# xymeng16/dcf

Hardware: AMD Instinct MI355X
Metric: DCF evals/sec (node) at 128-bit input, λ=16B; AES blocks/s vs INT roofline (higher is better)
Workload: dtype u8

## Files before the change

### dcf_amd/csrc/aes_lds.h

```cpp
#pragma once

namespace {

uint8_t g_sbox[256];
uint32_t g_tab[4 * 256];
std::once_flag g_aes_once;

uint8_t gmul(uint8_t a, uint8_t b) {
  uint8_t r = 0;
  for (; b; b >>= 1) {
    if (b & 1) r ^= a;
    a = (uint8_t)((a << 1) ^ ((a & 0x80) ? 0x1b : 0));
  }
  return r;
}

void aes_init_tables() {
  uint8_t exp_t[256], log_t[256] = {0};
  uint8_t x = 1;
  for (int i = 0; i < 255; i++) {
    exp_t[i] = x;
    log_t[x] = (uint8_t)i;
    x = gmul(x, 3);
  }
  for (int v = 0; v < 256; v++) {
    uint8_t inv = v ? exp_t[(255 - log_t[v]) % 255] : 0;
    uint8_t s = inv;
    for (int k = 1; k <= 4; k++) s ^= (uint8_t)((inv << k) | (inv >> (8 - k)));
    g_sbox[v] = (uint8_t)(s ^ 0x63);
  }
  for (int v = 0; v < 256; v++) {
    uint32_t s = g_sbox[v], s2 = gmul((uint8_t)s, 2), s3 = gmul((uint8_t)s, 3);
    uint32_t t0 = s2 | (s << 8) | (s << 16) | (s3 << 24);
    for (int t = 0; t < 4; t++) g_tab[t * 256 + v] = t ? ((t0 << (8 * t)) | (t0 >> (32 - 8 * t))) : t0;
  }
}

struct RoundKeys {
  uint32_t w[60];
};

void aes256_expand_words(const uint8_t key[32], RoundKeys* rk) {
  uint8_t b[240];
  memcpy(b, key, 32);
  uint8_t rcon = 1;
  for (int i = 8; i < 60; i++) {
    uint8_t t[4] = {b[4 * i - 4], b[4 * i - 3], b[4 * i - 2], b[4 * i - 1]};
    if (i % 8 == 0) {
      uint8_t t0 = t[0];
      t[0] = (uint8_t)(g_sbox[t[1]] ^ rcon);
      t[1] = g_sbox[t[2]];
      t[2] = g_sbox[t[3]];
      t[3] = g_sbox[t0];
      rcon = gmul(rcon, 2);
    } else if (i % 8 == 4) {
      for (auto& c : t) c = g_sbox[c];
    }
    for (int k = 0; k < 4; k++) b[4 * i + k] = (uint8_t)(b[4 * (i - 8) + k] ^ t[k]);
  }
  for (int i = 0; i < 60; i++)
    rk->w[i] = (uint32_t)b[4 * i] | ((uint32_t)b[4 * i + 1] << 8) | ((uint32_t)b[4 * i + 2] << 16) |
               ((uint32_t)b[4 * i + 3] << 24);
}

void aes128_expand_words(const uint8_t key[16], uint32_t w[44]) {
  uint8_t b[176];
  memcpy(b, key, 16);
  uint8_t rcon = 1;
  for (int i = 4; i < 44; i++) {
    uint8_t t[4] = {b[4 * i - 4], b[4 * i - 3], b[4 * i - 2], b[4 * i - 1]};
    if (i % 4 == 0) {
      const uint8_t t0 = t[0];
      t[0] = (uint8_t)(g_sbox[t[1]] ^ rcon);
      t[1] = g_sbox[t[2]];
      t[2] = g_sbox[t[3]];
      t[3] = g_sbox[t0];
      rcon = gmul(rcon, 2);
    }
    for (int k = 0; k < 4; k++) b[4 * i + k] = (uint8_t)(b[4 * (i - 4) + k] ^ t[k]);
  }
  for (int i = 0; i < 44; i++)
    w[i] = (uint32_t)b[4 * i] | ((uint32_t)b[4 * i + 1] << 8) | ((uint32_t)b[4 * i + 2] << 16) |
           ((uint32_t)b[4 * i + 3] << 24);
}

constexpr int kLdsWords = 32768;
constexpr int kBlock = 1024;
constexpr uint32_t kMaskLast = 0xFEFFFFFFu;

__device__ __forceinline__ void lds_fill_tables(uint32_t* lds, const uint32_t* __restrict__ tab) {
  for (int idx = threadIdx.x; idx < kLdsWords; idx += blockDim.x) {
    const int half = idx >> 14, rem = idx & 16383;
    const int b = rem >> 6, slot = rem & 63;
    lds[idx] = tab[(2 * half + (slot >> 5)) * 256 + b];
  }
  __syncthreads();
}

__device__ __forceinline__ uint32_t lane_const() {
  const uint32_t l = (threadIdx.x & 31u) * 4u;
  return l | ((128u + l) << 8) | (1u << 16);
}

template <int T, int K>
struct Sel {
  static constexpr uint32_t v =
      ((T & 1) ? 1u : 0u) | ((4u + K) << 8) | (((T >> 1) ? 2u : 0x0cu) << 16) | (0x0cu << 24);
};

#ifndef DCF_T1_BITOP3
#define DCF_T1_BITOP3 1
#endif
template <int T, int K, bool B1 = true>
__device__ __forceinline__ uint32_t lk(const uint32_t* lds, uint32_t w, uint32_t lc) {
  uint32_t addr;
  if (DCF_T1_BITOP3 && B1 && T == 1 && K == 1) {
    addr = __builtin_amdgcn_bitop3_b32(w, 0xFF00u, (lc >> 8) & 0xFFu, 0xEA);
  } else {
    addr = __builtin_amdgcn_perm(w, lc, Sel<T, K>::v);
  }
  return *reinterpret_cast<const uint32_t*>(reinterpret_cast<const char*>(lds) + addr);
}

constexpr int kQpRot1 = 1 | (2 << 2) | (3 << 4) | (0 << 6);
constexpr int kQpRot2 = 2 | (3 << 2) | (0 << 4) | (1 << 6);
constexpr int kQpRot3 = 3 | (0 << 2) | (1 << 4) | (2 << 6);
constexpr int kQpBcast0 = 0;

__device__ __forceinline__ uint32_t xor3(uint32_t a, uint32_t b, uint32_t c) {
  return __builtin_amdgcn_bitop3_b32(a, b, c, 0x96);
}

template <int NB>
__device__ __forceinline__ void aes256_tt(uint32_t (&st)[NB][4], const RoundKeys& rk, const uint32_t* lds,
                                          uint32_t lc) {
#pragma unroll
  for (int b = 0; b < NB; ++b)
#pragma unroll
    for (int j = 0; j < 4; ++j) st[b][j] ^= rk.w[j];
#pragma unroll
  for (int r = 1; r < 14; ++r) {
    uint32_t o[NB][4];
#pragma unroll
    for (int b = 0; b < NB; ++b)
#pragma unroll
      for (int j = 0; j < 4; ++j) {
        const uint32_t a = lk<0, 0>(lds, st[b][j], lc);
        const uint32_t c = lk<1, 1>(lds, st[b][(j + 1) & 3], lc);
        const uint32_t d = lk<2, 2>(lds, st[b][(j + 2) & 3], lc);
        const uint32_t e = lk<3, 3>(lds, st[b][(j + 3) & 3], lc);
        o[b][j] = xor3(xor3(a, c, d), e, rk.w[4 * r + j]);
      }
#pragma unroll
    for (int b = 0; b < NB; ++b)
#pragma unroll
      for (int j = 0; j < 4; ++j) st[b][j] = o[b][j];
  }
  uint32_t o[NB][4];
#pragma unroll
  for (int b = 0; b < NB; ++b)
#pragma unroll
    for (int j = 0; j < 4; ++j) {
      const uint32_t a = lk<2, 0>(lds, st[b][j], lc);
      const uint32_t c = lk<3, 1>(lds, st[b][(j + 1) & 3], lc);
      const uint32_t d = lk<0, 2>(lds, st[b][(j + 2) & 3], lc);
      const uint32_t e = lk<1, 3>(lds, st[b][(j + 3) & 3], lc);
      const uint32_t lo = __builtin_amdgcn_perm(c, a, 0x0c0c0500u);
      const uint32_t hi = __builtin_amdgcn_perm(e, d, 0x07020c0cu);
      o[b][j] = xor3(lo, hi, rk.w[56 + j]);
    }
#pragma unroll
  for (int b = 0; b < NB; ++b)
#pragma unroll
    for (int j = 0; j < 4; ++j) st[b][j] = o[b][j];
}

typedef unsigned int u32x4_t __attribute__((ext_vector_type(4)));
__device__ __forceinline__ uint4 lds_load16(uint32_t a) {
  const u32x4_t v = *(__attribute__((address_space(3))) const u32x4_t*)(size_t)a;
  return make_uint4(v.x, v.y, v.z, v.w);
}

template <int NR, int NB, bool PRE, int KR = 0>
__device__ __forceinline__ void aes_tt_lka(uint32_t (&st)[NB][4], const uint32_t (&ka)[NB], const uint32_t* lds,
                                           uint32_t lc, const uint32_t (*rkr)[2][4] = nullptr,
                                           const uint32_t* hm = nullptr) {
  if (!PRE) {
#pragma unroll
    for (int b = 0; b < NB; ++b) {
      const uint4 k = lds_load16(ka[b]);
      st[b][0] ^= k.x; st[b][1] ^= k.y; st[b][2] ^= k.z; st[b][3] ^= k.w;
    }
  }
#pragma unroll
  for (int r = 1; r <= NR; ++r) {
    uint32_t o[NB][4];
#pragma unroll
    for (int b = 0; b < NB; ++b) {
      uint32_t kw[4];
      if (r < KR) {
#pragma unroll
        for (int j = 0; j < 4; ++j) kw[j] = __builtin_amdgcn_bitop3_b32(hm[b], rkr[r][1][j], rkr[r][0][j], 0xCA);
      } else {
        const uint4 k = lds_load16(ka[b] + 16u * r);
        kw[0] = k.x; kw[1] = k.y; kw[2] = k.z; kw[3] = k.w;
      }
#pragma unroll
      for (int j = 0; j < 4; ++j) {
        if (r < NR) {
          const uint32_t a = lk<0, 0, false>(lds, st[b][j], lc);
          const uint32_t c = lk<1, 1, false>(lds, st[b][(j + 1) & 3], lc);
          const uint32_t d = lk<2, 2, false>(lds, st[b][(j + 2) & 3], lc);
          const uint32_t e = lk<3, 3, false>(lds, st[b][(j + 3) & 3], lc);
          o[b][j] = xor3(xor3(a, c, d), e, kw[j]);
        } else {
          const uint32_t a = lk<2, 0>(lds, st[b][j], lc);
          const uint32_t c = lk<3, 1>(lds, st[b][(j + 1) & 3], lc);
          const uint32_t d = lk<0, 2>(lds, st[b][(j + 2) & 3], lc);
          const uint32_t e = lk<1, 3>(lds, st[b][(j + 3) & 3], lc);
          o[b][j] = xor3(__builtin_amdgcn_perm(c, a, 0x0c0c0500u), __builtin_amdgcn_perm(e, d, 0x07020c0cu), kw[j]);
        }
      }
    }
#pragma unroll
    for (int b = 0; b < NB; ++b)
#pragma unroll
      for (int j = 0; j < 4; ++j) st[b][j] = o[b][j];
  }
}

template <int NR, int NB, bool LATE_KEYS = false>
__device__ __forceinline__ void aes_tt_lk(uint32_t (&st)[NB][4], const uint4* const (&rk)[NB], const uint32_t* lds,
                                          uint32_t lc) {
#pragma unroll
  for (int b = 0; b < NB; ++b) {
    const uint4 k = rk[b][0];
    st[b][0] ^= k.x; st[b][1] ^= k.y; st[b][2] ^= k.z; st[b][3] ^= k.w;
  }
#pragma unroll
  for (int r = 1; r < NR; ++r) {
    uint32_t o[NB][4];
#pragma unroll
    for (int b = 0; b < NB; ++b) {
      uint32_t z = 0u;
      if (LATE_KEYS) asm volatile("" : "+v"(z) : "v"(st[b][0]));
      const uint4 k = rk[b][r + z];
      const uint32_t kw[4] = {k.x, k.y, k.z, k.w};
#pragma unroll
      for (int j = 0; j < 4; ++j) {
        const uint32_t a = lk<0, 0>(lds, st[b][j], lc);
        const uint32_t c = lk<1, 1>(lds, st[b][(j + 1) & 3], lc);
        const uint32_t d = lk<2, 2>(lds, st[b][(j + 2) & 3], lc);
        const uint32_t e = lk<3, 3>(lds, st[b][(j + 3) & 3], lc);
        o[b][j] = xor3(xor3(a, c, d), e, kw[j]);
      }
    }
#pragma unroll
    for (int b = 0; b < NB; ++b)
#pragma unroll
      for (int j = 0; j < 4; ++j) st[b][j] = o[b][j];
  }
  uint32_t o[NB][4];
#pragma unroll
  for (int b = 0; b < NB; ++b) {
    const uint4 k = rk[b][NR];
    const uint32_t kw[4] = {k.x, k.y, k.z, k.w};
#pragma unroll
    for (int j = 0; j < 4; ++j) {
      const uint32_t a = lk<2, 0>(lds, st[b][j], lc);
      const uint32_t c = lk<3, 1>(lds, st[b][(j + 1) & 3], lc);
      const uint32_t d = lk<0, 2>(lds, st[b][(j + 2) & 3], lc);
      const uint32_t e = lk<1, 3>(lds, st[b][(j + 3) & 3], lc);
      const uint32_t lo = __builtin_amdgcn_perm(c, a, 0x0c0c0500u);
      const uint32_t hi = __builtin_amdgcn_perm(e, d, 0x07020c0cu);
      o[b][j] = xor3(lo, hi, kw[j]);
    }
  }
#pragma unroll
  for (int b = 0; b < NB; ++b)
#pragma unroll
    for (int j = 0; j < 4; ++j) st[b][j] = o[b][j];
}

template <int NB, bool PRE = false>
__device__ __forceinline__ void aes256_tt_gk(uint32_t (&st)[NB][4], const uint4* __restrict__ rkg,
                                             const uint32_t* lds, uint32_t lc) {
  const char* base = reinterpret_cast<const char*>(rkg);
  uint32_t zb = 0u;
  if (!PRE) {
    const uint4 k = *reinterpret_cast<const uint4*>(base);
#pragma unroll
    for (int b = 0; b < NB; ++b) {
      st[b][0] ^= k.x; st[b][1] ^= k.y; st[b][2] ^= k.z; st[b][3] ^= k.w;
    }
  }
  constexpr int AH = 3;
  uint4 kq[AH];
#pragma unroll
  for (int q = 0; q < AH - 1; ++q) kq[q] = *reinterpret_cast<const uint4*>(base + 16 * (q + 1));
#pragma unroll
  for (int r = 1; r < 15; ++r) {
    asm volatile("" : "+v"(zb) : "v"(st[0][0]), "v"(st[NB - 1][0]));
    const int rn = r + AH - 1;
    if (rn < 15) kq[(rn - 1) % AH] = *reinterpret_cast<const uint4*>(base + zb + 16 * rn);
    const uint4 k = kq[(r - 1) % AH];
    const uint32_t kw[4] = {k.x, k.y, k.z, k.w};
    uint32_t o[NB][4];
    if (r < 14) {
#pragma unroll
      for (int b = 0; b < NB; ++b)
#pragma unroll
        for (int j = 0; j < 4; ++j) {
          const uint32_t a = lk<0, 0>(lds, st[b][j], lc);
          const uint32_t c = lk<1, 1>(lds, st[b][(j + 1) & 3], lc);
          const uint32_t d = lk<2, 2>(lds, st[b][(j + 2) & 3], lc);
          const uint32_t e = lk<3, 3>(lds, st[b][(j + 3) & 3], lc);
          o[b][j] = xor3(xor3(a, c, d), e, kw[j]);
        }
    } else {
#pragma unroll
      for (int b = 0; b < NB; ++b)
#pragma unroll
        for (int j = 0; j < 4; ++j) {
          const uint32_t a = lk<2, 0>(lds, st[b][j], lc);
          const uint32_t c = lk<3, 1>(lds, st[b][(j + 1) & 3], lc);
          const uint32_t d = lk<0, 2>(lds, st[b][(j + 2) & 3], lc);
          const uint32_t e = lk<1, 3>(lds, st[b][(j + 3) & 3], lc);
          const uint32_t lo = __builtin_amdgcn_perm(c, a, 0x0c0c0500u);
          const uint32_t hi = __builtin_amdgcn_perm(e, d, 0x07020c0cu);
          o[b][j] = xor3(lo, hi, kw[j]);
        }
    }
#pragma unroll
    for (int b = 0; b < NB; ++b)
#pragma unroll
      for (int j = 0; j < 4; ++j) st[b][j] = o[b][j];
  }
}

template <int NB>
__device__ __forceinline__ void aes128_tt(uint32_t (&st)[NB][4], const uint4* const (&rk)[NB], const uint32_t* lds,
                                          uint32_t lc) {
  aes_tt_lk<10, NB>(st, rk, lds, lc);
}

#ifdef DCF_CLOCK_STAMPS
constexpr uint32_t kClkSlots = 8, kClkGroups = 4096;
__device__ unsigned long long g_clk_stamps[kClkSlots * kClkGroups * 4];
__device__ __forceinline__ void clk_stamp(uint32_t slot, uint32_t phase) {
  const uint32_t wg = blockIdx.x + gridDim.x * blockIdx.y;
  if (threadIdx.x == 0 && wg < kClkGroups) {
    const unsigned long long t = __builtin_amdgcn_s_memtime(), r = __builtin_amdgcn_s_memrealtime();
    unsigned long long* o = g_clk_stamps + ((size_t)slot * kClkGroups + wg) * 4 + 2 * phase;
    __hip_atomic_store(o, t, __ATOMIC_RELAXED, __HIP_MEMORY_SCOPE_AGENT);
    __hip_atomic_store(o + 1, r, __ATOMIC_RELAXED, __HIP_MEMORY_SCOPE_AGENT);
  }
}
#define DCF_CLK(slot, phase) clk_stamp(slot, phase)
#else
#define DCF_CLK(slot, phase)
#endif

__device__ __forceinline__ uint32_t bswap32(uint32_t x) { return __builtin_amdgcn_perm(x, x, 0x00010203u); }

__device__ __forceinline__ uint32_t load_bits32(const uint8_t* __restrict__ p, uint32_t c, uint32_t nbytes) {
  if ((nbytes & 3u) == 0) return bswap32(*reinterpret_cast<const uint32_t*>(p + 4 * c));
  uint32_t w = 0;
#pragma unroll
  for (int k = 0; k < 4; ++k) {
    const uint32_t idx = 4 * c + k;
    w = (w << 8) | (idx < nbytes ? (uint32_t)p[idx] : 0u);
  }
  return w;
}

}
```

### dcf_amd/csrc/kernels_stream.h

```cpp
#pragma once

#include "aes_lds.h"
#include "kernels16.h"

namespace {

__device__ __forceinline__ uint32_t dequeue_unit(uint32_t* ctr) {
  uint32_t u = 0;
  if ((threadIdx.x & 63u) == 0) u = atomicAdd(ctr, 1u);
  return __builtin_amdgcn_readfirstlane(u);
}

constexpr uint32_t kStreamUnit = 256;

__device__ __forceinline__ uint32_t lane_rank(uint64_t mask) {
  return __builtin_amdgcn_mbcnt_hi((uint32_t)(mask >> 32), __builtin_amdgcn_mbcnt_lo((uint32_t)mask, 0u));
}

template <int NS, bool XREG, bool MULTI>
struct StreamLane {
  uint32_t s[NS][4], v[NS][4], t[NS], ph[NS], lev[NS], cur[NS];
  uint32_t xw[NS][4];
  bool fresh[NS];
  const uint8_t* xp[NS];
  uint32_t ci[NS], pt[NS];
  bool alive[NS];
};

template <int NS, bool XREG, bool MULTI>
__device__ __forceinline__ void stream_load_x(StreamLane<NS, XREG, MULTI>& L, int i, const uint8_t* row,
                                              uint32_t nbytes) {
  if (nbytes == 16) {
    const uint4 x = *reinterpret_cast<const uint4*>(row);
    L.xw[i][0] = x.x; L.xw[i][1] = x.y; L.xw[i][2] = x.z; L.xw[i][3] = x.w;
  } else {
#pragma unroll
    for (int w = 0; w < 4; ++w) L.xw[i][w] = (4u * w < nbytes) ? reinterpret_cast<const uint32_t*>(row)[w] : 0u;
  }
}

template <int NS, bool XREG, bool MULTI, bool PFX = false, int NBC = 0, bool XLOADED = false, bool PK2 = false>
__device__ __forceinline__ void stream_start(StreamLane<NS, XREG, MULTI>& L, int i, uint64_t p,
                                             const uint4* __restrict__ s0s, const uint4 s0v, uint32_t party,
                                             const uint8_t* __restrict__ xs, uint32_t nbytes_rt, uint64_t ppk,
                                             const PrefixTable& pf) {
  const uint32_t nbytes = NBC ? (uint32_t)NBC : nbytes_rt;
  const uint32_t k = !MULTI ? 0u : PK2 ? (uint32_t)p >> __builtin_ctz((uint32_t)ppk) : (uint32_t)p / (uint32_t)ppk;
  const uint8_t* row = xs + p * nbytes;
  uint32_t w0;
  if (XREG) {
    if (!XLOADED) stream_load_x(L, i, row, nbytes);
    w0 = bswap32(L.xw[i][0]);
  } else {
    L.xp[i] = row;
    w0 = load_bits32(row, 0, nbytes);
  }
  uint32_t lev0 = 0u;
  if (PFX || pf.levels) {
    lev0 = pf.levels;
    uint4 sv, vv;
    const uint32_t top = w0 >> (32u - lev0);
    prefix_row(pf, MULTI ? (k << lev0) + top : top, sv, vv, L.t[i]);
    L.s[i][0] = sv.x; L.s[i][1] = sv.y; L.s[i][2] = sv.z; L.s[i][3] = sv.w;
    L.v[i][0] = vv.x; L.v[i][1] = vv.y; L.v[i][2] = vv.z; L.v[i][3] = vv.w;
  } else {
    const uint4 sv = MULTI ? s0s[k] : s0v;
    L.s[i][0] = sv.x; L.s[i][1] = sv.y; L.s[i][2] = sv.z; L.s[i][3] = sv.w;
#pragma unroll
    for (int j = 0; j < 4; ++j) L.v[i][j] = 0u;
    L.t[i] = party;
  }
  L.ph[i] = 0u;
  L.lev[i] = lev0;
  L.ci[i] = (uint32_t)k * (8u * nbytes) + lev0;
  L.pt[i] = (uint32_t)p;
  L.alive[i] = true;
  if (XREG) {
    if (PFX || lev0) {
      L.cur[i] = w0 << lev0;
      L.xw[i][0] = L.xw[i][1]; L.xw[i][1] = L.xw[i][2]; L.xw[i][2] = L.xw[i][3];
      L.fresh[i] = false;
    } else {
      L.fresh[i] = true;
    }
  } else {
    L.cur[i] = w0 << lev0;
  }
}

template <int NS, bool XREG, bool MULTI, uint32_t UNIT = kStreamUnit, bool PFX = false, int NBC = 0, bool PK2 = false>
__device__ __forceinline__ void stream_refill(StreamLane<NS, XREG, MULTI>& L, int i, bool mine, uint32_t& unext,
                                              uint32_t& uend, bool& exhausted, uint32_t* __restrict__ ctr,
                                              uint32_t nunits, uint32_t total, const uint4* __restrict__ s0s,
                                              const uint4 s0v, uint32_t party, const uint8_t* __restrict__ xs,
                                              uint32_t nbytes, uint64_t ppk, const PrefixTable& pf) {
  uint64_t need = __ballot(mine);
  constexpr bool ONCE = !MULTI && NBC != 0;
  if (ONCE) {
    uint32_t pnew = 0;
    bool got = false;
    while (need) {
      if (unext >= uend && !exhausted) {
        const uint32_t u = dequeue_unit(ctr);
        if (u >= nunits) {
          exhausted = true;
        } else {
          unext = u * UNIT;
          uend = min(unext + UNIT, total);
        }
      }
      if (exhausted && unext >= uend) break;
      const uint32_t rank = lane_rank(need);
      const bool take = mine && rank < uend - unext;
      pnew = take ? unext + rank : pnew;
      got = got || take;
      const uint64_t taken = __ballot(take);
      unext += (uint32_t)__popcll(taken);
      need &= ~taken;
      mine = mine && !take;
    }
    if (got) {
      stream_start<NS, XREG, MULTI, PFX, NBC, false, PK2>(L, i, pnew, s0s, s0v, party, xs, nbytes, ppk, pf);
    } else if (mine) {
      L.alive[i] = false;
      L.ci[i] = 0;
      L.lev[i] = 0;
    }
    return;
  }
  while (need) {
    if (unext >= uend && !exhausted) {
      const uint32_t u = dequeue_unit(ctr);
      if (u >= nunits) {
        exhausted = true;
      } else {
        unext = u * UNIT;
        uend = min(unext + UNIT, total);
      }
    }
    if (exhausted && unext >= uend) {
      if (mine) {
        L.alive[i] = false;
        L.ci[i] = 0;
        L.lev[i] = 0;
      }
      return;
    }
    const uint32_t rank = lane_rank(need);
    const bool take = mine && rank < uend - unext;
    if (take)
      stream_start<NS, XREG, MULTI, PFX, NBC, false, PK2>(L, i, unext + rank, s0s, s0v, party, xs, nbytes, ppk, pf);
    const uint64_t taken = __ballot(take);
    unext += (uint32_t)__popcll(taken);
    need &= ~taken;
    mine = mine && !take;
  }
}

template <int NS, bool XREG, bool MULTI>
__device__ __forceinline__ void stream_next_word(StreamLane<NS, XREG, MULTI>& L, int i, uint32_t nl, uint32_t nlev,
                                                 uint32_t nbytes) {
  if (XREG) {
    L.cur[i] = bswap32(L.xw[i][0]);
    L.xw[i][0] = L.xw[i][1];
    L.xw[i][1] = L.xw[i][2];
    L.xw[i][2] = L.xw[i][3];
  } else if (nl < nlev) {
    L.cur[i] = load_bits32(L.xp[i], nl >> 5, nbytes);
  }
}

constexpr uint32_t kKmKeys = 32, kKmLevs = 16, kKmThreads = 256;
__global__ __launch_bounds__(kKmThreads) void k_cw_keymajor(const uint4* __restrict__ cw_s,
                                                            const uint4* __restrict__ cw_v,
                                                            const uint8_t* __restrict__ cw_t, const uint32_t nlev,
                                                            const uint64_t num_keys, uint4* __restrict__ dig,
                                                            uint8_t* __restrict__ dig_t) {
  constexpr uint32_t RW = 2 * kKmLevs + 1;
  constexpr uint32_t ITEMS = kKmKeys * kKmLevs, PER = (ITEMS + kKmThreads - 1) / kKmThreads;
  __shared__ uint4 sh[kKmKeys * RW];
  __shared__ uint8_t sht[kKmKeys * kKmLevs];
  const uint64_t k0 = (uint64_t)blockIdx.x * kKmKeys;
  const uint32_t l0 = blockIdx.y * kKmLevs;
  const uint32_t nk = (uint32_t)min<uint64_t>(kKmKeys, num_keys - k0), nl = min(kKmLevs, nlev - l0);
  uint4 vs[PER], vv[PER];
  uint32_t vt[PER];
#pragma unroll
  for (uint32_t j = 0; j < PER; ++j) {
    const uint32_t it = threadIdx.x + j * kKmThreads;
    const uint32_t l = it / kKmKeys, kk = it % kKmKeys;
    const bool ok = it < ITEMS && kk < nk && l < nl;
    const uint64_t src = ok ? (uint64_t)(l0 + l) * num_keys + k0 + kk : 0u;
    vs[j] = cw_s[src];
    vv[j] = cw_v[src];
    vt[j] = cw_t[src];
  }
#pragma unroll
  for (uint32_t j = 0; j < PER; ++j) {
    const uint32_t it = threadIdx.x + j * kKmThreads;
    if (it < ITEMS) {
      const uint32_t l = it / kKmKeys, kk = it % kKmKeys;
      sh[kk * RW + 2 * l] = vs[j];
      sh[kk * RW + 2 * l + 1] = vv[j];
      sht[kk * kKmLevs + l] = (uint8_t)vt[j];
    }
  }
  __syncthreads();
#pragma unroll
  for (uint32_t j = 0; j < (2 * ITEMS + kKmThreads - 1) / kKmThreads; ++j) {
    const uint32_t it = threadIdx.x + j * kKmThreads;
    const uint32_t kk = it / (2 * kKmLevs), r = it % (2 * kKmLevs);
    if (it < 2 * ITEMS && kk < nk && r < 2 * nl) dig[(k0 + kk) * nlev * 2 + 2 * l0 + r] = sh[kk * RW + r];
  }
#pragma unroll
  for (uint32_t j = 0; j < PER; ++j) {
    const uint32_t it = threadIdx.x + j * kKmThreads;
    const uint32_t kk = it / kKmLevs, l = it % kKmLevs;
    if (it < ITEMS && kk < nk && l < nl) dig_t[(k0 + kk) * nlev + l0 + l] = sht[kk * kKmLevs + l];
  }
}

#ifndef DCF_REUSE_RUN
#define DCF_REUSE_RUN 0
#endif
#ifndef DCF_STG_SLOTS
#define DCF_STG_SLOTS 2
#endif
constexpr int kStgH = DCF_STG_SLOTS;
static_assert(kStgH >= 2 && kStgH <= 32 && 64 % kStgH == 0, "DCF_STG_SLOTS: 2, 4, 8, 16 or 32");
constexpr uint32_t kStgUnit = 64 / kStgH;
constexpr uint32_t kStgBytes = kStgUnit * 32u;
__device__ __forceinline__ void glds16(const void* src, uint32_t lds_dst) {
  uint32_t keep;
  asm volatile("s_mov_b32 %0, m0\n\ts_mov_b32 m0, %2\n\ts_nop 0\n\tglobal_load_lds_dwordx4 %1, off\n\ts_mov_b32 m0, %0"
               : "=&s"(keep)
               : "v"(src), "s"(lds_dst)
               : "memory");
}

constexpr int kVmcnt0 = (0x7 << 4) | (0xF << 8);
#ifndef DCF_STG_PIN
#define DCF_STG_PIN 1
#endif
#ifndef DCF_STG_EARLY
#define DCF_STG_EARLY 1
#endif
#ifndef DCF_STREAM_PRIO
#define DCF_STREAM_PRIO 1
#endif
template <int NS, bool XREG, bool MULTI, uint32_t UNIT, bool GK, bool PFX = false, int NBC = 0, bool PK2 = false,
          bool STG = false>
__device__ __forceinline__ void stream_run(
    const uint32_t* lds, const uint4* rkl, const RoundKeys& rk, const uint4* __restrict__ cw_s,
    const uint4* __restrict__ cw_v, const uint8_t* __restrict__ cw_t, const uint4* __restrict__ cw_np1,
    const uint4* __restrict__ s0s, const uint32_t party, const uint8_t* __restrict__ xs, const uint32_t nbytes_rt,
    const uint64_t num_keys, const uint64_t ppk, const uint64_t total, uint32_t* __restrict__ ctr,
    uint4* __restrict__ ys, const PrefixTable& pf, const uint32_t stg_lds = 0u) {
  static_assert(!STG || (!MULTI && XREG && PFX && NBC > 0 && NBC <= 4),
                "staged rows: single key, prefix table, x in one word");
  const uint32_t nbytes = NBC ? (uint32_t)NBC : nbytes_rt;
  const uint32_t lc = lane_const();
  const uint32_t nlev = 8u * nbytes;
  const uint32_t total32 = (uint32_t)total;
  const uint32_t nunits = (uint32_t)((total + UNIT - 1) / UNIT);
  uint32_t unext = 0, uend = 0;
  bool exhausted = false;
  const uint4 s0v = s0s[0];
  StreamLane<NS, XREG, MULTI> L;
#pragma unroll
  for (int i = 0; i < NS; ++i) {
    L.fresh[i] = false;
    L.alive[i] = false;
    L.ci[i] = 0;
    L.lev[i] = 0;
    L.ph[i] = 0u;
  }
  const uint4 np1v = cw_np1[0];
  uint32_t hb[kStgH], hn[kStgH], hs[kStgH], hu[kStgH], xh[kStgH], xr[kStgH];
#pragma unroll
  for (int h = 0; h < kStgH; ++h) hb[h] = hn[h] = hs[h] = hu[h] = xh[h] = xr[h] = 0u;
  auto staged = [&]() {
    bool any = false;
#pragma unroll
    for (int h = 0; h < kStgH; ++h) any = any || hs[h] != 0u;
    return any;
  };
  const uint32_t lane = threadIdx.x & 63u;
  auto claim = [&](int h) {
    if (unext >= uend && !exhausted) {
      const uint32_t u = dequeue_unit(ctr);
      if (u >= nunits) {
        exhausted = true;
      } else {
        unext = u * UNIT;
        uend = min(unext + UNIT, total32);
      }
    }
    if (unext >= uend) return;
    hb[h] = unext;
    hn[h] = min(kStgUnit, uend - unext);
    unext += hn[h];
    hu[h] = 0u;
    const uint32_t pp = hb[h] + min(lane % kStgUnit, hn[h] - 1u);
    xh[h] = *reinterpret_cast<const uint32_t*>(xs + (size_t)pp * nbytes);
    hs[h] = 1u;
  };
  auto stage = [&]() {
#pragma unroll
    for (int h = 0; h < kStgH; ++h)
      if (hs[h] == 0u) claim(h);
#pragma unroll
    for (int h = 0; h < kStgH; ++h) {
      if (!DCF_STG_EARLY && hs[h] == 2u) {
        const uint32_t top = bswap32(xr[h]) >> (32u - pf.levels);
        if (lane < 2u * kStgUnit) glds16(pf.sv + 2u * top + lane / kStgUnit, stg_lds + kStgBytes * h);
        hs[h] = 3u;
      }
    }
#pragma unroll
    for (int h = 0; h < kStgH; ++h)
      if (hs[h] == 1u) hs[h] = 2u;
  };
  auto prep = [&]() {
    if (DCF_STG_EARLY) {
      bool out = false;
#pragma unroll
      for (int h = 0; h < kStgH; ++h) out = out || hs[h] == 4u;
      if (out) __builtin_amdgcn_s_waitcnt(kVmcnt0);
#pragma unroll
      for (int h = 0; h < kStgH; ++h)
        if (hs[h] == 4u) hs[h] = 3u;
    }
#pragma unroll
    for (int h = 0; h < kStgH; ++h) {
      if (hs[h] == 2u) {
        asm volatile("v_mov_b32 %0, %1" : "=v"(xr[h]) : "v"(xh[h]));
        if (DCF_STG_EARLY) {
          const uint32_t top = bswap32(xr[h]) >> (32u - pf.levels);
          if (lane < 2u * kStgUnit) glds16(pf.sv + 2u * top + lane / kStgUnit, stg_lds + kStgBytes * h);
          hs[h] = 4u;
        }
      }
    }
  };
  auto refill_stg = [&](int i, bool mine) {
    uint64_t need = __ballot(mine);
    asm volatile("" ::: "memory");
#pragma unroll
    for (int h = 0; h < kStgH; ++h) {
      if (need && hs[h] == 3u) {
        const uint32_t rank = lane_rank(need);
        const bool take = mine && rank < hn[h] - hu[h];
        const uint32_t r = min(hu[h] + rank, hn[h] - 1u);
        const uint32_t xw = (uint32_t)__builtin_amdgcn_ds_bpermute((int)(r << 2), (int)xr[h]);
        const uint4 sv = lds_load16(stg_lds + kStgBytes * h + 16u * r);
        const uint4 vv = lds_load16(stg_lds + kStgBytes * h + 16u * (kStgUnit + r));
        if (take) {
          const uint32_t lev0 = pf.levels;
          L.s[i][0] = sv.x; L.s[i][1] = sv.y; L.s[i][2] = sv.z; L.s[i][3] = sv.w & kMaskLast;
          L.v[i][0] = vv.x; L.v[i][1] = vv.y; L.v[i][2] = vv.z; L.v[i][3] = vv.w;
          L.t[i] = (sv.w >> 24) & 1u;
          L.ph[i] = 0u;
          L.lev[i] = lev0;
          L.ci[i] = lev0;
          L.pt[i] = hb[h] + r;
          L.alive[i] = true;
          L.cur[i] = bswap32(xw) << lev0;
          L.xw[i][0] = 0u; L.xw[i][1] = 0u; L.xw[i][2] = 0u;
          L.fresh[i] = false;
        }
        const uint64_t taken = __ballot(take);
        hu[h] += (uint32_t)__popcll(taken);
        need &= ~taken;
        mine = mine && !take;
        if (hu[h] == hn[h]) {
          hs[h] = 0u;
          claim(h);
        }
      }
    }
    if (need)
      stream_refill<NS, XREG, MULTI, UNIT, PFX, NBC, PK2>(L, i, mine, unext, uend, exhausted, ctr, nunits, total32,
                                                         s0s, s0v, party, xs, nbytes, ppk, pf);
  };
  if (STG) stage();
#pragma unroll
  for (int i = 0; i < NS; ++i)
    stream_refill<NS, XREG, MULTI, UNIT, PFX, NBC, PK2>(L, i, true, unext, uend, exhausted, ctr, nunits, total32,
                                                       s0s, s0v, party, xs, nbytes, ppk, pf);

  uint64_t nblk = 0;
  for (;;) {
    bool any = false;
#pragma unroll
    for (int i = 0; i < NS; ++i) {
      any = any || L.alive[i];
      nblk += (uint64_t)__popcll(__ballot(L.alive[i]));
    }
    const bool pend = STG && staged();
    if (!__ballot(any) && !pend) break;
    uint4 cs[NS], cv[NS], cs2[NS], cv2[NS];
    uint32_t ct[NS], ct2[NS];
    bool maybe[NS];
#pragma unroll
    for (int i = 0; i < NS; ++i) {
      const uint32_t cwi = MULTI ? L.ci[i] : L.lev[i];
      if (MULTI) {
        cs[i] = cw_s[2 * cwi];
        cv[i] = cw_s[2 * cwi + 1];
      } else {
        cs[i] = cw_s[cwi];
        cv[i] = cw_v[cwi];
      }
      ct[i] = cw_t[cwi];
      maybe[i] = L.alive[i] && L.ph[i] == 0u && L.t[i] == 0u && (!XREG || PFX || !L.fresh[i]) &&
                 (L.cur[i] >> 31) != 0u && L.lev[i] + 1u < nlev;
      const uint32_t c2 = cwi + (L.lev[i] + 1u < nlev ? 1u : 0u);
      if (MULTI) {
        cs2[i] = cw_s[2 * c2];
        cv2[i] = cw_s[2 * c2 + 1];
      } else {
        cs2[i] = cw_s[c2];
        cv2[i] = cw_v[c2];
      }
      ct2[i] = cw_t[c2];
    }
    uint32_t st[NS][4];
    uint4 k0 = make_uint4(0u, 0u, 0u, 0u);
    if (GK) k0 = rkl[0];
    const uint32_t k0w[4] = {k0.x, k0.y, k0.z, k0.w};
#pragma unroll
    for (int i = 0; i < NS; ++i) {
      const uint32_t inv = L.ph[i] - 1u;
#pragma unroll
      for (int j = 0; j < 4; ++j) st[i][j] = GK ? xor3(L.s[i][j], inv, k0w[j]) : (L.s[i][j] ^ inv);
    }
    if (DCF_STREAM_PRIO == 1) __builtin_amdgcn_s_setprio(1);
    if (DCF_STREAM_PRIO == 2) __builtin_amdgcn_s_setprio(0);
    if (GK)
      aes256_tt_gk<NS, true>(st, rkl, lds, lc);
    else
      aes256_tt<NS>(st, rk, lds, lc);
    if (DCF_STREAM_PRIO == 1) __builtin_amdgcn_s_setprio(0);
    if (DCF_STREAM_PRIO == 2) __builtin_amdgcn_s_setprio(1);
#pragma unroll
    for (int i = 0; i < NS; ++i)
      asm volatile("" : "+v"(cs[i].x), "+v"(cs[i].y), "+v"(cs[i].z), "+v"(cs[i].w), "+v"(cv[i].x), "+v"(cv[i].y),
                   "+v"(cv[i].z), "+v"(cv[i].w), "+v"(ct[i]));
#pragma unroll
    for (int i = 0; i < NS; ++i)
      asm volatile("" : "+v"(cs2[i].x), "+v"(cs2[i].y), "+v"(cs2[i].z), "+v"(cs2[i].w), "+v"(cv2[i].x),
                   "+v"(cv2[i].y), "+v"(cv2[i].z), "+v"(cv2[i].w), "+v"(ct2[i]));
#pragma unroll
    for (int i = 0; i < NS; ++i) {
      if (XREG && !PFX) {
        const bool nw = L.fresh[i];
        L.cur[i] = nw ? bswap32(L.xw[i][0]) : L.cur[i];
        L.xw[i][0] = nw ? L.xw[i][1] : L.xw[i][0];
        L.xw[i][1] = nw ? L.xw[i][2] : L.xw[i][1];
        L.xw[i][2] = nw ? L.xw[i][3] : L.xw[i][2];
        L.fresh[i] = false;
      }
      const uint32_t p = L.ph[i], xb = L.cur[i] >> 31;
      const uint32_t adv = L.alive[i] ? (p | xb) : 0u;
      const uint32_t inv = p - 1u;
      const uint32_t keepB = xb - 1u;
      const uint32_t tm = 0u - L.t[i], am = 0u - adv, pm = 0u - p;
      const uint32_t csw[4] = {cs[i].x, cs[i].y, cs[i].z, cs[i].w};
      const uint32_t cvw[4] = {cv[i].x, cv[i].y, cv[i].z, cv[i].w};
      uint32_t d[4];
#pragma unroll
      for (int j = 0; j < 4; ++j) d[j] = st[i][j] ^ L.s[i][j] ^ inv;
      const uint32_t d0 = d[0];
      const bool reuse = maybe[i] && (L.s[i][3] & ~kMaskLast) == 0u;
#pragma unroll
      for (int j = 0; j < 4; ++j) {
        const uint32_t msk = (j == 3) ? kMaskLast : 0xFFFFFFFFu;
        const uint32_t in = L.s[i][j] ^ inv;
        const uint32_t vhat = (in ^ (st[i][j] & keepB)) & msk;
        L.v[i][j] ^= inv & (vhat ^ (tm & cvw[j]));
        const uint32_t sx = L.s[i][j] ^ (st[i][j] & pm);
        const uint32_t sn = (sx & msk) ^ (tm & csw[j]);
        L.s[i][j] = (am & sn) | (~am & L.s[i][j]);
      }
      const uint32_t tb = (d0 ^ (L.t[i] & (ct[i] >> xb))) & 1u;
      L.t[i] = (am & tb) | (~am & L.t[i]);
      L.ph[i] = adv ^ 1u;
      uint32_t nl = L.lev[i] + adv;
      L.cur[i] <<= adv;
      if (!(NBC && NBC <= 4) && adv && (nl & 31u) == 0u) stream_next_word<NS, XREG, MULTI>(L, i, nl, nlev, nbytes);
      L.ci[i] += adv;
      {
        const uint32_t xb2 = L.cur[i] >> 31, t1 = L.t[i], tm1 = 0u - t1;
        const uint32_t rm = 0u - (uint32_t)reuse, rr = rm & (0u - xb2);
        const uint32_t cs2w[4] = {cs2[i].x, cs2[i].y, cs2[i].z, cs2[i].w};
        const uint32_t cv2w[4] = {cv2[i].x, cv2[i].y, cv2[i].z, cv2[i].w};
#pragma unroll
        for (int j = 0; j < 4; ++j) {
          const uint32_t msk = (j == 3) ? kMaskLast : 0xFFFFFFFFu;
          L.v[i][j] ^= rm & ((((xb2 ? ~L.s[i][j] : d[j]) & msk) ^ (tm1 & cv2w[j])));
          L.s[i][j] ^= rr & tm1 & cs2w[j];
        }
        L.t[i] = rr ? ((d0 ^ (t1 & (ct2[i] >> 1))) & 1u) : L.t[i];
        L.ph[i] = (reuse && !xb2) ? 1u : L.ph[i];
        nl += rr & 1u;
        L.cur[i] <<= (rr & 1u);
        L.ci[i] += rr & 1u;
        if (!(NBC && NBC <= 4) && rr && (nl & 31u) == 0u) stream_next_word<NS, XREG, MULTI>(L, i, nl, nlev, nbytes);
        if (DCF_REUSE_RUN) {
          const bool go = rr && t1 == 0u && (nl & 31u) != 0u && nl < nlev;
          const uint32_t k = go ? min((uint32_t)__clz(~L.cur[i]), nlev - nl) : 0u;
          const uint32_t ko = 0u - (k & 1u);
          nl += k;
          L.cur[i] <<= k;
          L.ci[i] += k;
          const uint32_t lm = 0u - (uint32_t)(go && nl < nlev && (nl & 31u) != 0u);
#pragma unroll
          for (int j = 0; j < 4; ++j) {
            const uint32_t msk = (j == 3) ? kMaskLast : 0xFFFFFFFFu;
            L.v[i][j] ^= ((ko & ~L.s[i][j]) ^ (lm & d[j])) & msk;
          }
          L.ph[i] = lm ? 1u : L.ph[i];
          if (!(NBC && NBC <= 4) && go && k && (nl & 31u) == 0u && nl < nlev)
            stream_next_word<NS, XREG, MULTI>(L, i, nl, nlev, nbytes);
        }
      }
      L.lev[i] = nl;
    }
    if (STG) {
      if (DCF_STG_PIN)
#pragma unroll
        for (int i = 0; i < NS; ++i)
          asm volatile("" : "+v"(L.s[i][0]), "+v"(L.s[i][1]), "+v"(L.s[i][2]), "+v"(L.s[i][3]), "+v"(L.v[i][0]),
                       "+v"(L.v[i][1]), "+v"(L.v[i][2]), "+v"(L.v[i][3]), "+v"(L.t[i]));
      prep();
    }
#pragma unroll
    for (int i = 0; i < NS; ++i) {
      const bool done = L.alive[i] && L.lev[i] == nlev;
      if (done) {
        const uint32_t key = PK2 ? L.pt[i] >> __builtin_ctz((uint32_t)ppk) : L.pt[i] / (uint32_t)ppk;
        const uint4 np = MULTI ? cw_np1[key] : np1v;
        const uint32_t tm = 0u - L.t[i];
        ys[L.pt[i]] = make_uint4(L.v[i][0] ^ L.s[i][0] ^ (tm & np.x), L.v[i][1] ^ L.s[i][1] ^ (tm & np.y),
                                 L.v[i][2] ^ L.s[i][2] ^ (tm & np.z), L.v[i][3] ^ L.s[i][3] ^ (tm & np.w));
      }
      if (STG) {
        const bool want = done || (!L.alive[i] && staged());
        if (__ballot(want)) refill_stg(i, want);
      } else if (__ballot(done)) {
        stream_refill<NS, XREG, MULTI, UNIT, PFX, NBC, PK2>(L, i, done, unext, uend, exhausted, ctr, nunits, total32,
                                                           s0s, s0v, party, xs, nbytes, ppk, pf);
      }
    }
    if (STG) stage();
  }
  if ((threadIdx.x & 63u) == 0) atomicAdd(reinterpret_cast<unsigned long long*>(ctr) + 1, (unsigned long long)nblk);
}

template <int NS, bool XREG, bool MULTI, bool PFX = false, int NBC = 0, bool PK2 = false, bool STG = false>
__global__ __launch_bounds__(kBlock, 1) void k_eval16_stream(
    const uint32_t* __restrict__ tab, const RoundKeys rk, const uint4* __restrict__ cw_s,
    const uint4* __restrict__ cw_v, const uint8_t* __restrict__ cw_t, const uint4* __restrict__ cw_np1,
    const uint4* __restrict__ s0s, const uint32_t party, const uint8_t* __restrict__ xs, const uint32_t nbytes,
    const uint64_t num_keys, const uint64_t ppk, const uint64_t total, uint32_t* __restrict__ ctr,
    uint4* __restrict__ ys, const PrefixTable pf, const uint4* __restrict__ rkg) {
  __shared__ uint32_t lds[kLdsWords];
  lds_fill_tables(lds, tab);
  DCF_CLK(2, 0);
#ifndef DCF_STG_GK
#define DCF_STG_GK 1
#endif
  constexpr bool GK = (!STG || DCF_STG_GK) && (!MULTI || (!PFX && XREG));
  if constexpr (STG) {
    __shared__ uint4 stg[kBlock / 64 * 128];
    const uint32_t stg_lds = __builtin_amdgcn_readfirstlane(
        (uint32_t)(size_t)(__attribute__((address_space(3))) uint4*)stg + (threadIdx.x >> 6) * 2048u);
    stream_run<NS, XREG, MULTI, kStreamUnit, GK, PFX, NBC, PK2, STG>(
        lds, rkg, rk, cw_s, cw_v, cw_t, cw_np1, s0s, party, xs, nbytes, num_keys, ppk, total, ctr, ys, pf, stg_lds);
  } else {
    stream_run<NS, XREG, MULTI, kStreamUnit, GK, PFX, NBC, PK2>(lds, rkg, rk, cw_s, cw_v, cw_t, cw_np1, s0s, party,
                                                               xs, nbytes, num_keys, ppk, total, ctr, ys, pf);
  }
  DCF_CLK(2, 1);
}

}
```

Baseline: 562.4 million.

## Rewrite DCF stream level update with bitop3 masks and enable reuse runs by default

Rewrites the per-level state update in the streaming DCF evaluator as fused three-input bitop3 operations on precomputed masks. The separate reuse step and run-skip step are merged into one k-level advance, and run-length skipping is now on by default for every kernel variant. Single-key correction-word loads now use byte offsets from the level index, and the maybe[] predicate array is dropped. This is meant to cut VALU instruction count and allow more levels to be skipped without an AES call. The risk is subtle mask bugs in the merged logic and extra register pressure.

```diff
diff --git a/dcf_amd/csrc/aes_lds.h b/dcf_amd/csrc/aes_lds.h
--- a/dcf_amd/csrc/aes_lds.h
+++ b/dcf_amd/csrc/aes_lds.h
@@ -131,6 +131,17 @@
   return __builtin_amdgcn_bitop3_b32(a, b, c, 0x96);
 }
 
+constexpr uint32_t kTa = 0xF0u, kTb = 0xCCu, kTc = 0xAAu;
+template <uint32_t TT>
+__device__ __forceinline__ uint32_t bop3(uint32_t a, uint32_t b, uint32_t c) {
+  return __builtin_amdgcn_bitop3_b32(a, b, c, TT & 0xFFu);
+}
+constexpr uint32_t kTtXorAnd = kTa ^ (kTb & kTc);
+constexpr uint32_t kTtXorAndNot = kTa ^ (kTb & ~kTc);
+constexpr uint32_t kTtSel = (kTa & ~kTc) | (kTb & kTc);
+constexpr uint32_t kTtAndOr = kTa & (kTb | kTc);
+constexpr uint32_t kTtAndNotNot = kTa & ~kTb & ~kTc;
+
 template <int NB>
 __device__ __forceinline__ void aes256_tt(uint32_t (&st)[NB][4], const RoundKeys& rk, const uint32_t* lds,
                                           uint32_t lc) {
diff --git a/dcf_amd/csrc/kernels_stream.h b/dcf_amd/csrc/kernels_stream.h
--- a/dcf_amd/csrc/kernels_stream.h
+++ b/dcf_amd/csrc/kernels_stream.h
@@ -220,8 +220,23 @@
   }
 }
 
-#ifndef DCF_REUSE_RUN
-#define DCF_REUSE_RUN 0
+#ifdef DCF_REUSE_RUN
+#define DCF_REUSE_RUN_SK DCF_REUSE_RUN
+#define DCF_REUSE_RUN_SK4 DCF_REUSE_RUN
+#define DCF_REUSE_RUN_MK DCF_REUSE_RUN
+#define DCF_REUSE_RUN_XW DCF_REUSE_RUN
+#endif
+#ifndef DCF_REUSE_RUN_XW
+#define DCF_REUSE_RUN_XW 1
+#endif
+#ifndef DCF_REUSE_RUN_SK
+#define DCF_REUSE_RUN_SK 1
+#endif
+#ifndef DCF_REUSE_RUN_SK4
+#define DCF_REUSE_RUN_SK4 1
+#endif
+#ifndef DCF_REUSE_RUN_MK
+#define DCF_REUSE_RUN_MK 1
 #endif
 #ifndef DCF_STG_SLOTS
 #define DCF_STG_SLOTS 2
@@ -259,6 +274,7 @@
   static_assert(!STG || (!MULTI && XREG && PFX && NBC > 0 && NBC <= 4),
                 "staged rows: single key, prefix table, x in one word");
   const uint32_t nbytes = NBC ? (uint32_t)NBC : nbytes_rt;
+  constexpr bool RUN = !XREG ? DCF_REUSE_RUN_XW : MULTI ? DCF_REUSE_RUN_MK : (NBC && NBC <= 4) ? DCF_REUSE_RUN_SK4 : DCF_REUSE_RUN_SK;
   const uint32_t lc = lane_const();
   const uint32_t nlev = 8u * nbytes;
   const uint32_t total32 = (uint32_t)total;
@@ -401,29 +417,29 @@
     if (!__ballot(any) && !pend) break;
     uint4 cs[NS], cv[NS], cs2[NS], cv2[NS];
     uint32_t ct[NS], ct2[NS];
-    bool maybe[NS];
 #pragma unroll
     for (int i = 0; i < NS; ++i) {
-      const uint32_t cwi = MULTI ? L.ci[i] : L.lev[i];
       if (MULTI) {
+        const uint32_t cwi = L.ci[i];
+        const uint32_t c2 = cwi + (L.lev[i] + 1u < nlev ? 1u : 0u);
         cs[i] = cw_s[2 * cwi];
         cv[i] = cw_s[2 * cwi + 1];
-      } else {
-        cs[i] = cw_s[cwi];
-        cv[i] = cw_v[cwi];
-      }
-      ct[i] = cw_t[cwi];
-      maybe[i] = L.alive[i] && L.ph[i] == 0u && L.t[i] == 0u && (!XREG || PFX || !L.fresh[i]) &&
-                 (L.cur[i] >> 31) != 0u && L.lev[i] + 1u < nlev;
-      const uint32_t c2 = cwi + (L.lev[i] + 1u < nlev ? 1u : 0u);
-      if (MULTI) {
+        ct[i] = cw_t[cwi];
         cs2[i] = cw_s[2 * c2];
         cv2[i] = cw_s[2 * c2 + 1];
+        ct2[i] = cw_t[c2];
       } else {
-        cs2[i] = cw_s[c2];
-        cv2[i] = cw_v[c2];
-      }
-      ct2[i] = cw_t[c2];
+        const uint32_t off = L.lev[i] << 4;
+        const uint8_t* ps = reinterpret_cast<const uint8_t*>(cw_s) + off;
+        const uint8_t* pv = reinterpret_cast<const uint8_t*>(cw_v) + off;
+        const uint8_t* pt = cw_t + L.lev[i];
+        cs[i] = *reinterpret_cast<const uint4*>(ps);
+        cv[i] = *reinterpret_cast<const uint4*>(pv);
+        ct[i] = pt[0];
+        cs2[i] = *reinterpret_cast<const uint4*>(ps + 16);
+        cv2[i] = *reinterpret_cast<const uint4*>(pv + 16);
+        ct2[i] = pt[1];
+      }
     }
     uint32_t st[NS][4];
     uint4 k0 = make_uint4(0u, 0u, 0u, 0u);
@@ -453,78 +469,78 @@
                    "+v"(cv2[i].y), "+v"(cv2[i].z), "+v"(cv2[i].w), "+v"(ct2[i]));
 #pragma unroll
     for (int i = 0; i < NS; ++i) {
+      uint32_t fm = 0u;
       if (XREG && !PFX) {
         const bool nw = L.fresh[i];
+        fm = nw ? ~0u : 0u;
         L.cur[i] = nw ? bswap32(L.xw[i][0]) : L.cur[i];
         L.xw[i][0] = nw ? L.xw[i][1] : L.xw[i][0];
         L.xw[i][1] = nw ? L.xw[i][2] : L.xw[i][1];
         L.xw[i][2] = nw ? L.xw[i][3] : L.xw[i][2];
         L.fresh[i] = false;
       }
-      const uint32_t p = L.ph[i], xb = L.cur[i] >> 31;
-      const uint32_t adv = L.alive[i] ? (p | xb) : 0u;
-      const uint32_t inv = p - 1u;
-      const uint32_t keepB = xb - 1u;
-      const uint32_t tm = 0u - L.t[i], am = 0u - adv, pm = 0u - p;
+      const uint32_t pm = 0u - L.ph[i];
+      const uint32_t xm = (uint32_t)((int32_t)L.cur[i] >> 31);
+      const uint32_t tm = 0u - L.t[i];
+      const uint32_t am = bop3<kTtAndOr>(L.alive[i] ? ~0u : 0u, pm, xm);
+      const uint32_t adv = am & 1u;
+      const uint32_t inv = ~pm;
+      const uint32_t ik = ~(pm | xm);
+      const uint32_t itm = tm & ~pm, apm = am & pm, atm = am & tm;
+      const uint32_t ikw[4] = {ik, ik, ik, ik & kMaskLast};
+      const uint32_t invw[4] = {inv, inv, inv, inv & kMaskLast};
+      const uint32_t apmw[4] = {apm, apm, apm, apm & kMaskLast};
       const uint32_t csw[4] = {cs[i].x, cs[i].y, cs[i].z, cs[i].w};
       const uint32_t cvw[4] = {cv[i].x, cv[i].y, cv[i].z, cv[i].w};
+      const uint32_t s3bad = (uint32_t)__builtin_amdgcn_sbfe((int)L.s[i][3], 24u, 1u);
+      const uint32_t rm = bop3<kTtAndNotNot>(bop3<kTtAndNotNot>(am, pm, tm), s3bad, fm);
       uint32_t d[4];
 #pragma unroll
-      for (int j = 0; j < 4; ++j) d[j] = st[i][j] ^ L.s[i][j] ^ inv;
+      for (int j = 0; j < 4; ++j) d[j] = xor3(st[i][j], L.s[i][j], inv);
       const uint32_t d0 = d[0];
-      const bool reuse = maybe[i] && (L.s[i][3] & ~kMaskLast) == 0u;
 #pragma unroll
       for (int j = 0; j < 4; ++j) {
-        const uint32_t msk = (j == 3) ? kMaskLast : 0xFFFFFFFFu;
-        const uint32_t in = L.s[i][j] ^ inv;
-        const uint32_t vhat = (in ^ (st[i][j] & keepB)) & msk;
-        L.v[i][j] ^= inv & (vhat ^ (tm & cvw[j]));
-        const uint32_t sx = L.s[i][j] ^ (st[i][j] & pm);
-        const uint32_t sn = (sx & msk) ^ (tm & csw[j]);
-        L.s[i][j] = (am & sn) | (~am & L.s[i][j]);
-      }
-      const uint32_t tb = (d0 ^ (L.t[i] & (ct[i] >> xb))) & 1u;
-      L.t[i] = (am & tb) | (~am & L.t[i]);
-      L.ph[i] = adv ^ 1u;
+        uint32_t vj = bop3<kTtXorAnd>(L.v[i][j], st[i][j], ikw[j]);
+        vj = bop3<kTtXorAndNot>(vj, invw[j], L.s[i][j]);
+        L.v[i][j] = bop3<kTtXorAnd>(vj, cvw[j], itm);
+        uint32_t sj = L.s[i][j];
+        if (j == 3) sj &= ~am | kMaskLast;
+        sj = bop3<kTtXorAnd>(sj, st[i][j], apmw[j]);
+        L.s[i][j] = bop3<kTtXorAnd>(sj, csw[j], atm);
+      }
+      const uint32_t tb = bop3<kTtXorAnd>(d0, L.t[i], ct[i] >> (xm & 1u));
+      L.t[i] = bop3<kTtSel>(L.t[i], tb, adv);
       uint32_t nl = L.lev[i] + adv;
       L.cur[i] <<= adv;
       if (!(NBC && NBC <= 4) && adv && (nl & 31u) == 0u) stream_next_word<NS, XREG, MULTI>(L, i, nl, nlev, nbytes);
-      L.ci[i] += adv;
-      {
-        const uint32_t xb2 = L.cur[i] >> 31, t1 = L.t[i], tm1 = 0u - t1;
-        const uint32_t rm = 0u - (uint32_t)reuse, rr = rm & (0u - xb2);
-        const uint32_t cs2w[4] = {cs2[i].x, cs2[i].y, cs2[i].z, cs2[i].w};
-        const uint32_t cv2w[4] = {cv2[i].x, cv2[i].y, cv2[i].z, cv2[i].w};
-#pragma unroll
-        for (int j = 0; j < 4; ++j) {
-          const uint32_t msk = (j == 3) ? kMaskLast : 0xFFFFFFFFu;
-          L.v[i][j] ^= rm & ((((xb2 ? ~L.s[i][j] : d[j]) & msk) ^ (tm1 & cv2w[j])));
-          L.s[i][j] ^= rr & tm1 & cs2w[j];
-        }
-        L.t[i] = rr ? ((d0 ^ (t1 & (ct2[i] >> 1))) & 1u) : L.t[i];
-        L.ph[i] = (reuse && !xb2) ? 1u : L.ph[i];
-        nl += rr & 1u;
-        L.cur[i] <<= (rr & 1u);
-        L.ci[i] += rr & 1u;
-        if (!(NBC && NBC <= 4) && rr && (nl & 31u) == 0u) stream_next_word<NS, XREG, MULTI>(L, i, nl, nlev, nbytes);
-        if (DCF_REUSE_RUN) {
-          const bool go = rr && t1 == 0u && (nl & 31u) != 0u && nl < nlev;
-          const uint32_t k = go ? min((uint32_t)__clz(~L.cur[i]), nlev - nl) : 0u;
-          const uint32_t ko = 0u - (k & 1u);
-          nl += k;
-          L.cur[i] <<= k;
-          L.ci[i] += k;
-          const uint32_t lm = 0u - (uint32_t)(go && nl < nlev && (nl & 31u) != 0u);
-#pragma unroll
-          for (int j = 0; j < 4; ++j) {
-            const uint32_t msk = (j == 3) ? kMaskLast : 0xFFFFFFFFu;
-            L.v[i][j] ^= ((ko & ~L.s[i][j]) ^ (lm & d[j])) & msk;
-          }
-          L.ph[i] = lm ? 1u : L.ph[i];
-          if (!(NBC && NBC <= 4) && go && k && (nl & 31u) == 0u && nl < nlev)
-            stream_next_word<NS, XREG, MULTI>(L, i, nl, nlev, nbytes);
-        }
-      }
+      const uint32_t t1 = L.t[i], tm1 = 0u - t1;
+      const uint32_t ones = RUN ? (uint32_t)__clz((int)~L.cur[i]) : L.cur[i] >> 31;
+      const uint32_t klim = RUN ? (bop3<kTa & (kTb ^ kTc)>(rm, tm1, 32u) & 33u) : (rm & 1u);
+      const uint32_t k = min(min(ones, nlev - nl), klim);
+      const uint32_t ko = (uint32_t)__builtin_amdgcn_sbfe((int)k, 0u, 1u);
+      nl += k;
+      L.cur[i] <<= k;
+      const bool cross = k != 0u && (nl & 31u) == 0u;
+      const uint32_t below = (uint32_t)((int32_t)(nl - nlev) >> 31);
+      const uint32_t xm2 = (uint32_t)((int32_t)L.cur[i] >> 31);
+      const uint32_t lm0 = bop3<kTtAndNotNot>(rm & below, xm2, RUN ? (tm1 & ko) : ko);
+      const uint32_t lm = cross ? 0u : lm0;
+      const uint32_t vm2 = bop3<kTtAndOr>(tm1, ko, lm), sm = tm1 & ko;
+      const uint32_t kow[4] = {ko, ko, ko, ko & kMaskLast};
+      const uint32_t lmw[4] = {lm, lm, lm, lm & kMaskLast};
+      const uint32_t cs2w[4] = {cs2[i].x, cs2[i].y, cs2[i].z, cs2[i].w};
+      const uint32_t cv2w[4] = {cv2[i].x, cv2[i].y, cv2[i].z, cv2[i].w};
+#pragma unroll
+      for (int j = 0; j < 4; ++j) {
+        uint32_t vj = bop3<kTtXorAndNot>(L.v[i][j], kow[j], L.s[i][j]);
+        vj = bop3<kTtXorAnd>(vj, d[j], lmw[j]);
+        L.v[i][j] = bop3<kTtXorAnd>(vj, cv2w[j], vm2);
+        L.s[i][j] = bop3<kTtXorAnd>(L.s[i][j], cs2w[j], sm);
+      }
+      L.t[i] = bop3<kTtSel>(t1, d0 ^ (ct2[i] >> 1), sm & 1u);
+      L.ph[i] = bop3<kTa | (kTb & kTc)>(adv ^ 1u, lm, 1u);
+      if (!(NBC && NBC <= 4) && cross) stream_next_word<NS, XREG, MULTI>(L, i, nl, nlev, nbytes);
+      if (MULTI) L.ci[i] += adv + k;
       L.lev[i] = nl;
     }
     if (STG) {
```

After: 595.2 million (median of 6 runs). 5.8% higher.
